# davidlougheed/strkit

Hardware: AMD Instinct MI355X
Metric: reads/sec realigned (higher is better)
Workload: dtype int32; 1 GPU; cfg2 shape (1000 loci x 30 HiFi reads, motif 3-6 bp, flank 70), 10000 loci x 30 reads per step and GPU, 8 distinct resident batches in rotation; exact scores (banded first pass with exactness certificate, exact fall-back); distinct_batches=8, parallelism=loci-sharded x1, calls_in_flight=2

## Files before the change

### strkit_amd/csrc/strk_api.hip

```cpp
#include "strk_host.h"
#include "strk_policy.h"
#include "strk_groups.h"
#include "strk_phase_check.h"
#include "strk_phase_inputs.h"
#include "strk_methyl.h"

#include <algorithm>
#include <array>
#include <atomic>
#include <chrono>
#include <cmath>
#include <condition_variable>
#include <cstdlib>
#include <cstring>
#include <memory>
#include <mutex>
#include <thread>
#include <vector>
#include <fcntl.h>
#include <sched.h>
#include <sys/stat.h>
#include <unistd.h>

#include "strk_kernels.h"
#include "strk_realign.h"
#include "strk_frontend.h"
#include "strk_inflate.h"
#include "strk_alleles.h"
#include "strk_phase.h"
#include "strk_consensus.h"
#include "strk_kmers.h"
#include "strk_poa.h"

namespace {

struct HostPipe;

std::atomic<int> g_calls_in_flight{0};

strk_policy::WindowPolicy g_window;
static_assert(strk_policy::kWinBuckets == strk::kWinBuckets, "strk_policy.h <-> strk_kernels.h");
static_assert(strk_groups::kInvalid == STRK_E_INVALID, "strk_groups.h <-> include/strkit_amd.h");
static_assert(strk_realign_plan::kNoMem == STRK_E_NOMEM, "strk_realign_plan.h <-> include/strkit_amd.h");

std::mutex g_band_chain_mu;
hipEvent_t g_band_chain_ev = nullptr;
int g_band_chain_dev = -1;

int host_cpus() {
    cpu_set_t set;
    CPU_ZERO(&set);
    if (sched_getaffinity(0, sizeof set, &set) == 0 && CPU_COUNT(&set) > 0) return CPU_COUNT(&set);
    return std::max(1u, std::thread::hardware_concurrency());
}

constexpr size_t kCellsOff = 64 * sizeof(int32_t);
constexpr size_t kCountersBytes = kCellsOff + 10 * sizeof(unsigned long long);
constexpr int kU64ScratchUsed = 1, kU64BandBytes = 2, kU64ExactBytes = 3, kU64WideBytes = 4, kU64LongBytes = 5;
constexpr size_t kWideHistOff = (kCountersBytes + 63) & ~(size_t)63;
constexpr size_t kCountersAllBytes = kWideHistOff + 2 * strk::kNumWideLists * 256 * sizeof(int32_t);

struct HostCounters {
    PinnedBuf mem;
    int cnt(int k) const { return mem.as<const int32_t>()[k]; }
    unsigned long long u64(int k) const { return reinterpret_cast<const unsigned long long*>(mem.as<const char>() + kCellsOff)[k]; }
    unsigned long long cells() const { return u64(0); }
    unsigned long long cells_of(int k_cell) const { return u64(k_cell); }
    unsigned long long scratch_used() const { return u64(kU64ScratchUsed); }
    unsigned long long band_bytes() const { return u64(kU64BandBytes); }
    unsigned long long exact_bytes() const { return u64(kU64ExactBytes); }
    unsigned long long wide_bytes() const { return u64(kU64WideBytes); }
    unsigned long long long_bytes() const { return u64(kU64LongBytes); }
    int band_reads() const {
        int n = 0;
        for (int k = 0; k < strk::kNumBandClasses; ++k) n += cnt(strk::kCntClass0 + strk::kBandClass0 + k);
        return n;
    }
};

struct GroupStage {
    DevBuf off, start, len, seqs;
    const uint8_t* bases = nullptr;
    int upload(const strk_groups::View& v, const strk_groups::Totals& t, const uint8_t* h_seqs, const uint8_t* d_seqs, hipStream_t st) {
        const size_t ng = (size_t)v.n_groups, ns = (size_t)t.n_seqs;
        int rc;
        if ((rc = off.ensure((ng + 1) * 4))) return rc;
        if ((rc = start.ensure(std::max<size_t>(ns, 1) * 8))) return rc;
        if ((rc = len.ensure(std::max<size_t>(ns, 1) * 4))) return rc;
        if (!d_seqs && (rc = seqs.ensure(std::max<size_t>((size_t)v.n_seq_bytes, 256)))) return rc;
        bases = d_seqs ? d_seqs : seqs.as<uint8_t>();
        if (!d_seqs && t.total_len > 0) HIP_TRY(hipMemcpyAsync(seqs.p, h_seqs, (size_t)v.n_seq_bytes, hipMemcpyHostToDevice, st));
        HIP_TRY(hipMemcpyAsync(off.p, v.group_off, (ng + 1) * 4, hipMemcpyHostToDevice, st));
        if (ns > 0) {
            HIP_TRY(hipMemcpyAsync(start.p, v.seq_start, ns * 8, hipMemcpyHostToDevice, st));
            HIP_TRY(hipMemcpyAsync(len.p, v.seq_len, ns * 4, hipMemcpyHostToDevice, st));
        }
        return 0;
    }
};

}

struct strk_ctx {
    int device = 0;
    int last_list_stride = 0;
    DevBuf read_locus, win_lo, win_n, tab_off, table, cls_list, band_recs, band_recs_w, long_list, counters, scratch, state_i32, state_f64, spec, rhash, rep, exact;
    DevBuf win_lo2, win_n2, tab_off2, table2, items;
    DevBuf stage_in, stage_out;
    PinnedBuf sc_host, sc_out;
    DevBuf rl_call, rl_chunk;
    Stream side;
    DevBuf al_in, al_ws, al_out;
    DevBuf ph_in, ph_mid, ph_ws, ph_out;
    GroupStage cs_in;
    DevBuf cs_bound, cs_out;
    GroupStage km_in;
    DevBuf km_k, km_cnt, km_eoff, km_list, km_slist, km_wsoff, km_ws, km_out;
    GroupStage po_in;
    DevBuf po_res, po_pool, po_poolof, po_list, po_ws, po_out, po_outoff;
    HostCounters h_counters;
    Event ev[9];
    size_t scratch_ints = 0;
    size_t long_slot_ints = 0, generic_ints = 0;
    strk_policy::BandGate band;
    strk_policy::GridHistory hist;
    bool p_window_auto = false;
    int p_window_b[strk::kWinBuckets] = {0, 0, 0, 0, 0};
    bool pending = false;
    strk_batch p_batch;
    strk_params p_params;
    strk_params p_params_in;
    int scratch_reruns = 0;
    strk::KArgs p_args;
    strk::ReplayArgs p_replay;
    hipStream_t p_stream = nullptr;
    HostPipe* pipe = nullptr;
};

namespace {

using namespace strk;

constexpr int kDefaultWindow = 8;
enum { kEvStart = 0, kEvHead, kEvBand, kEvWide, kEvPre, kEvExact, kEvLong, kEvGeneric, kEvEnd, kNumEvents };
constexpr int kBandProbationReads = 2048;
constexpr int kBandSpanW = 64, kBandSlackM8 = 0, kBandSpanMaxMotif = 6;
constexpr int kBandBlocksPerCU = std::max(1, std::min(8, (160 * 1024) / (4 * kBandWaveLds + kLdsSlack + 1024)));
constexpr int kLongBlocks = 512, kLongWaves = kLongBlocks * 4;
constexpr size_t kLongSlotInts = (size_t)48 << 10;
constexpr size_t kGenericPoolInts = (size_t)16 << 20;
constexpr size_t kLongSlotMaxInts = (size_t)kLongTile * kLongMaxTiles + 2 * (((size_t)1 << 20) + 256);
constexpr unsigned long long kGenericPoolMaxInts = 8ull << 30;
int check_params(const strk_params* p, strk_params* out) {
    if (!p) return fail(STRK_E_INVALID, "params is NULL");
    *out = *p;
    if (out->window <= 0) out->window = kDefaultWindow;
    if (2 * out->window + 1 > kTableMax) out->window = (kTableMax - 1) / 2;
    if (out->local_search_range < 0 || out->step_size < 1)
        return fail(STRK_E_INVALID, "local_search_range must be >= 0 and step_size >= 1");
    if (out->tie_rule != STRK_TIE_FIRST && out->tie_rule != STRK_TIE_LAST) return fail(STRK_E_INVALID, "bad tie_rule");
    if (out->end_flags < 0 || out->end_flags > 15) return fail(STRK_E_INVALID, "bad end_flags");
    static_assert(STRK_NARROW_NONE == strk::kNarrowNone && STRK_NARROW_DECREMENT == strk::kNarrowDecrement &&
                  STRK_NARROW_HALVE == strk::kNarrowHalve && STRK_NARROW_AFTER_SEED == strk::kNarrowAfterSeed, "include/strkit_amd.h <-> strk_search.h");
    if (out->narrowing < 0 || out->narrowing >= strk::kNarrowModes)
        return fail(STRK_E_INVALID, "narrowing schedule %d is not one of STRK_NARROW_NONE / _DECREMENT / _HALVE / _AFTER_SEED", out->narrowing);
    return 0;
}

int ensure_workspace(strk_ctx* c, int n_reads, int n_loci, size_t table_ints, size_t n_items) {
    const size_t nr = (size_t)std::max(n_reads, 1), nl = (size_t)std::max(n_loci, 1);
    int rc;
    if ((rc = c->read_locus.ensure(nr * 4))) return rc;
    if ((rc = c->win_lo.ensure(nr * 4))) return rc;
    if ((rc = c->win_n.ensure(nr * 4))) return rc;
    if ((rc = c->tab_off.ensure(nr * 8))) return rc;
    if ((rc = c->table.ensure(std::max<size_t>(table_ints, 1) * 4))) return rc;
    if ((rc = c->cls_list.ensure((size_t)kNumLists * std::max<size_t>(n_items, 1) * 2 * 4))) return rc;
    if ((rc = c->band_recs.ensure((size_t)kNumBandClasses * std::max<size_t>(n_items, 1) * 3 * sizeof(int4)))) return rc;
    if ((rc = c->counters.ensure(kCountersAllBytes))) return rc;
    if ((rc = c->band_recs_w.ensure((size_t)kNumBandClasses * std::max<size_t>(n_items, 1) * 3 * sizeof(int4)))) return rc;
    if ((rc = c->state_i32.ensure(nl * 4 * 4))) return rc;
    if ((rc = c->state_f64.ensure(nl * 8))) return rc;
    if ((rc = c->spec.ensure(nr * 16))) return rc;
    if ((rc = c->rhash.ensure(nr * 8))) return rc;
    if ((rc = c->rep.ensure(nr * 4))) return rc;
    if ((rc = c->exact.ensure(nr))) return rc;
    if (!c->scratch.p) {
        if ((rc = c->scratch.ensure(((size_t)kLongWaves * c->long_slot_ints + c->generic_ints) * 4))) return rc;
        c->scratch_ints = (size_t)kLongWaves * c->long_slot_ints + c->generic_ints;
    }
    return 0;
}

KArgs make_args(strk_ctx* c, const strk_batch* b, int end_flags, int window, int table_stride, int list_stride,
                const strk_params* sp) {
    KArgs a;
    memset(&a, 0, sizeof a);
    a.seqs = b->seqs; a.seq_off = b->seq_off; a.nfl = b->nfl; a.ntr = b->ntr; a.nfr = b->nfr;
    a.est_cn = b->est_cn; a.read_off = b->read_off; a.motifs = b->motifs; a.motif_off = b->motif_off;
    a.n_reads = b->n_reads; a.n_loci = b->n_loci;
    a.read_locus = c->read_locus.as<int32_t>();
    a.win_lo = c->win_lo.as<int32_t>();
    a.win_n = c->win_n.as<int32_t>();
    a.tab_off = c->tab_off.as<int64_t>();
    a.table = c->table.as<int32_t>();
    a.cls_list = c->cls_list.as<int32_t>();
    a.band_recs = c->band_recs.as<int4>();
    a.band_recs_w = a.band_recs;
    a.wide_hist = reinterpret_cast<int32_t*>(c->counters.as<char>() + kWideHistOff);
    a.counters = c->counters.as<int32_t>();
    a.cells = reinterpret_cast<unsigned long long*>(c->counters.as<char>() + kCellsOff);
    a.scratch_used = a.cells + 1;
    a.scratch = c->scratch.as<int32_t>();
    a.scratch_cap = (long long)c->scratch_ints;
    a.long_slot = (long long)c->long_slot_ints;
    a.long_waves = kLongWaves;
    a.list_stride = list_stride;
    c->last_list_stride = list_stride;
    a.band_tune = {kBandSpanW, kBandSlackM8, kBandSpanMaxMotif};
    a.end_flags = end_flags;
    a.window = window;
    for (int k = 0; k < kWinBuckets; ++k) a.window_b[k] = c->p_window_b[k] > 0 ? c->p_window_b[k] : window;
    a.table_stride = table_stride;
    if (sp) {
        a.spec = static_cast<int4*>(c->spec.p);
        a.max_iters = sp->max_iters; a.lsr = sp->local_search_range; a.step = sp->step_size;
        a.tie_last = sp->tie_rule == STRK_TIE_LAST;
        a.narrow = sp->narrowing;
        a.rep = c->rep.as<int32_t>();
        a.rhash = sp->no_dedupe ? nullptr : c->rhash.as<unsigned long long>();
        a.exact = c->exact.as<uint8_t>();
        a.band_mode = (!sp->no_band && c->band.cooldown == 0) ? 1 : 0;
        a.band_limit = c->band.probation ? kBandProbationReads : INT32_MAX;
    }
    return a;
}

void enqueue_scoring(strk_ctx* c, const KArgs& a, int mode, const int32_t* d_items, int n_items, int force_generic,
                     hipStream_t st, bool time_dp, const ReplayArgs* pre_replay = nullptr) {
    const bool hist = c->hist.usable(mode, a.band_mode);
    const bool sort_wide = a.band_mode && mode == 0 && !force_generic && (!hist || (c->hist.wide_chunks > 0 && c->hist.wide_chunks <= 8192));
    const int plan_scope = plan_scope_of(n_items);
    hipLaunchKernelGGL(k_plan, dim3((n_items + plan_scope - 1) / plan_scope), dim3(kPlanThreads), 0, st, a, mode, d_items, n_items, force_generic,
                       plan_reads_per_thread(n_items));
    const bool overlap = g_calls_in_flight.load(std::memory_order_relaxed) > 1;
    const bool heavy = c->hist.valid && c->hist.tail_heavy;
    const int sixteenths = (overlap && !heavy) ? 15 : 16;
    auto predicted_blocks = [&](int chunks, int full) { return c->hist.predicted_blocks(hist, chunks, a.n_reads, full); };
    if (time_dp) (void)hipEventRecord(c->ev[kEvHead], st);
    const bool band = a.band_mode && mode == 0 && !force_generic;
    int band_blocks = 1;
    if (band && time_dp) {
        std::lock_guard<std::mutex> lk(g_band_chain_mu);
        if (sixteenths == 16 && overlap && g_band_chain_ev && g_band_chain_ev != c->ev[kEvBand].h && g_band_chain_dev == c->device)
            (void)hipStreamWaitEvent(st, g_band_chain_ev, 0);
    }
    if (band) {
        band_blocks = std::max(1, std::min(256 * kBandBlocksPerCU * sixteenths / 16, (a.list_stride + 3) / 4));
        hipLaunchKernelGGL(k_dp_band, dim3(band_blocks), dim3(256), 0, st, a);
    }
    if (time_dp) (void)hipEventRecord(c->ev[kEvBand], st);
    if (band && time_dp) {
        std::lock_guard<std::mutex> lk(g_band_chain_mu);
        g_band_chain_ev = c->ev[kEvBand].h;
        g_band_chain_dev = c->device;
    }
    if (band) {
        KArgs aw = a;
        if (sort_wide) {
            hipLaunchKernelGGL(k_sort_wide_hist, dim3(kSortWideBlocks, kNumWideLists), dim3(256), 0, st, a);
            hipLaunchKernelGGL(k_sort_wide, dim3(kSortWideBlocks, kNumWideLists), dim3(256), 0, st, a, c->band_recs_w.as<int4>());
            aw.band_recs_w = c->band_recs_w.as<int4>();
        }
        const int wide_full = std::max(1, std::min(256 * kBandBlocksPerCU * sixteenths / 16, (a.list_stride + 3) / 4));
        hipLaunchKernelGGL(k_dp_band_wide, dim3(predicted_blocks(c->hist.wide_chunks, wide_full)), dim3(256), 0, st, aw);
    }
    if (time_dp) (void)hipEventRecord(c->ev[kEvWide], st);
    if (band && pre_replay) hipLaunchKernelGGL(k_replay, dim3(a.n_loci), dim3(64), 0, st, a, *pre_replay);
    if (time_dp) (void)hipEventRecord(c->ev[kEvPre], st);
    if (!force_generic) {
        constexpr int kBlocksPerCU = std::max(1, std::min(8, (160 * 1024) / (4 * kWaveLdsBytes + kLdsSlack + 1024)));
        const int full = std::max(1, std::min(256 * kBlocksPerCU * sixteenths / 16, (a.list_stride + 3) / 4));
        const int blocks = a.ref_mode ? full : predicted_blocks(c->hist.exact_chunks, full);
        if (a.ref_mode) hipLaunchKernelGGL(k_dp_ref, dim3(blocks), dim3(256), 0, st, a);
        else hipLaunchKernelGGL(k_dp_all, dim3(blocks), dim3(256), 0, st, a);
    }
    if (time_dp) (void)hipEventRecord(c->ev[kEvExact], st);
    KArgs al = a;
    if (!force_generic && !a.ref_mode) {
        const bool many_long = mode == 0 ? (!hist || c->hist.n_long > kLongWaves) : a.list_stride > kLongWaves;
        if (many_long && !c->long_list.ensure((size_t)std::max(1, a.list_stride) * 2 * 4)) {
            hipLaunchKernelGGL(k_sort_long, dim3(1), dim3(1024), 0, st, a, c->long_list.as<int32_t>());
            al.long_sorted = c->long_list.as<int32_t>();
        }
    }
    if (!force_generic && !a.ref_mode)
        hipLaunchKernelGGL(k_dp_long, dim3(mode == 0 ? predicted_blocks(c->hist.n_long, kLongBlocks) : std::max(1, std::min(kLongBlocks, a.list_stride))),
                           dim3(256), 0, st, al);
    if (time_dp) (void)hipEventRecord(c->ev[kEvLong], st);
    hipLaunchKernelGGL(k_dp_generic, dim3(1024), dim3(256), 0, st, a);
    if (time_dp) (void)hipEventRecord(c->ev[kEvGeneric], st);
}

// ... 30 lines not shown

int score_until_scratch_fits(strk_ctx* c, KArgs& a, const int32_t* d_items, int n_items, int force_generic, hipStream_t st,
                             bool timed, KArgs* outer = nullptr, void* copy_dst = nullptr, const void* copy_src = nullptr,
                             size_t copy_bytes = 0) {
    for (int attempt = 0;; ++attempt) {
        HIP_TRY(hipMemsetAsync(c->counters.p, 0, kCountersBytes, st));
        if (timed) HIP_TRY(hipEventRecord(c->ev[kEvStart], st));
        enqueue_scoring(c, a, 1, d_items, n_items, force_generic, st, timed);
        if (timed) HIP_TRY(hipEventRecord(c->ev[kEvEnd], st));
        HIP_TRY(hipMemcpyAsync(c->h_counters.mem.p, c->counters.p, kCountersBytes, hipMemcpyDeviceToHost, st));
        if (copy_bytes) HIP_TRY(hipMemcpyAsync(copy_dst, copy_src, copy_bytes, hipMemcpyDeviceToHost, st));
        HIP_TRY(hipStreamSynchronize(st));
        HIP_TRY(hipGetLastError());
        if (attempt >= 3 || !grow_scratch(c)) return 0;
        for (KArgs* k : {&a, outer}) {
            if (!k) continue;
            k->scratch = c->scratch.as<int32_t>();
            k->scratch_cap = (long long)c->scratch_ints;
            k->long_slot = (long long)c->long_slot_ints;
        }
    }
}

#include "strk_host_miss.inc"

int submit_device(strk_ctx* c, const strk_batch* b, const strk_params* params, int32_t* out_cn, int32_t* out_score,
                  int32_t* out_n, int32_t* out_start, hipStream_t st) {
    if (c->pending) return fail(STRK_E_INVALID, "context already holds a submitted call: strk_finish() it first");
    strk_params p;
    int rc;
    if ((rc = check_params(params, &p))) return rc;
    if (!b || b->n_reads < 0 || b->n_loci < 0) return fail(STRK_E_INVALID, "bad batch");
    c->p_window_auto = params->window <= 0;
    for (int k = 0; k < kWinBuckets; ++k) c->p_window_b[k] = 0;
    if (c->p_window_auto) {
        p.window = 0;
        for (int k = 0; k < kWinBuckets; ++k) {
            c->p_window_b[k] = g_window.window(k, p.local_search_range + p.step_size);
            p.window = std::max(p.window, c->p_window_b[k]);
        }
    }
    c->p_batch = *b;
    c->p_params = p;
    c->p_params_in = *params;
    c->p_stream = st;
    if (b->n_reads == 0 || b->n_loci == 0) {
        c->pending = true;
        g_calls_in_flight.fetch_add(1, std::memory_order_relaxed);
        return 0;
    }
    if (!out_cn || !out_score || !out_n || !out_start) return fail(STRK_E_INVALID, "output pointer is NULL");
    HIP_TRY(hipSetDevice(c->device));
    const int ts = std::min(kTableMax - 1, 2 * (p.window + 7) + 1);
    if ((rc = ensure_workspace(c, b->n_reads, b->n_loci, (size_t)b->n_reads * ts, (size_t)b->n_reads))) return rc;
    KArgs a = make_args(c, b, p.end_flags, p.window, ts, b->n_reads, &p);
    ReplayArgs rp;
    rp.max_iters = p.max_iters; rp.lsr = p.local_search_range; rp.step = p.step_size;
    rp.tie_last = p.tie_rule == STRK_TIE_LAST; rp.feedback = p.feedback; rp.narrow = p.narrowing;
    rp.out_cn = out_cn; rp.out_score = out_score; rp.out_n = out_n; rp.out_start = out_start;
    rp.next_read = c->state_i32.as<int32_t>();
    rp.need_lo = rp.next_read + b->n_loci;
    rp.need_hi = rp.need_lo + b->n_loci;
    rp.stop = rp.need_hi + b->n_loci;
    rp.frac = c->state_f64.as<double>();
    rp.resume = 0;
    rp.pre_exact = 0;

    struct InFlight {
        bool keep = false;
        InFlight() { g_calls_in_flight.fetch_add(1, std::memory_order_relaxed); }
        ~InFlight() { if (!keep) g_calls_in_flight.fetch_sub(1, std::memory_order_relaxed); }
    } in_flight;
    HIP_TRY(hipEventRecord(c->ev[kEvStart], st));
    HIP_TRY(hipMemsetAsync(c->counters.p, 0, kCountersAllBytes, st));
    if (a.rhash) hipLaunchKernelGGL(k_hash, dim3((b->n_reads + 31) / 32), dim3(256), 0, st, a);
    ReplayArgs rp_pre = rp;
    rp_pre.pre_exact = 1;
    enqueue_scoring(c, a, 0, nullptr, b->n_reads, 0, st, true, a.band_mode ? &rp_pre : nullptr);
    rp.resume = a.band_mode ? 1 : 0;
    hipLaunchKernelGGL(k_replay, dim3(b->n_loci), dim3(64), 0, st, a, rp);
    HIP_TRY(hipMemcpyAsync(c->h_counters.mem.p, c->counters.p, kCountersBytes, hipMemcpyDeviceToHost, st));
    HIP_TRY(hipEventRecord(c->ev[kEvEnd], st));
    HIP_TRY(hipGetLastError());
    c->p_args = a;
    c->p_replay = rp;
    c->pending = true;
    in_flight.keep = true;
    return 0;
}

void fill_stats(strk_ctx* c, const HostCounters& n, strk_stats* stats) {
    auto span = [&](int from, int to) {
        float ms = 0.f;
        return hipEventElapsedTime(&ms, c->ev[from], c->ev[to]) == hipSuccess ? ms : 0.f;
    };
    stats->kernel_ms = span(kEvStart, kEvEnd);
    stats->head_ms = span(kEvStart, kEvHead);
    stats->band_kernel_ms = span(kEvHead, kEvBand);
    stats->band_wide_kernel_ms = span(kEvBand, kEvWide);
    stats->dp_kernel_ms = span(kEvPre, kEvExact);
    stats->long_kernel_ms = span(kEvExact, kEvLong);
    stats->generic_kernel_ms = span(kEvLong, kEvGeneric);
    stats->replay_ms = span(kEvGeneric, kEvEnd) + span(kEvWide, kEvPre);
    stats->band_bytes = (int64_t)n.band_bytes();
    stats->exact_bytes = (int64_t)n.exact_bytes();
    stats->wide_bytes = (int64_t)n.wide_bytes();
    stats->long_bytes = (int64_t)n.long_bytes();
// ... 692 lines not shown
```

### strkit_amd/csrc/strk_dp_band.h

```cpp
#pragma once

namespace strk {

struct BandLayout {
    int wd, pad, maxdb, maxcol, off_sel, off_cp, cp_bytes, ct_bytes, cp_tail, off_ct, off_b0, group_bytes, sel_len;
    static constexpr int OFF_COMB = 0, OFF_MISC = OFF_COMB + kTableMax * 4, OFF_LMAX = OFF_MISC + 16;
    static constexpr int kBandHiPad = kBandRowSlack + 32;
    __host__ __device__ constexpr BandLayout(int c)
        : wd(128 << c), pad((128 << c) + (8 << c) + 8), maxdb(band_max_db(c)), maxcol(band_max_col(c)),
          off_sel(OFF_LMAX + (band_class_lmax(c) ? kTableMax * 4 : 0)),
          off_cp(off_sel + ((band_max_db(c) + 2 * ((128 << c) + (8 << c) + 8) + kBandHiPad + 15) & ~15)),
          cp_bytes(band_class_fly(c) ? 512 : ((band_max_db(c) + kBandRowSlack + 2 * (8 << c) + 4 + 15) & ~15)),
          ct_bytes((kBandMaxFlank + 2 * (8 << c) + 4 + 15) & ~15),
          cp_tail(c == 0 ? cp_bytes - ct_bytes : cp_bytes),
          off_ct(off_cp + cp_tail),
          off_b0(off_ct + ct_bytes),
          group_bytes(off_b0 + ((band_max_col(c) * 2 + 15) & ~15)),
          sel_len((band_max_db(c) + 2 * ((128 << c) + (8 << c) + 8) + kBandHiPad) & ~3) {}
};
static_assert(band_class_layout(4) == 0 && band_class_layout(7) == 3 && band_class_wd(5) <= band_class_wd(1) && band_class_G(6) == band_class_G(2),
              "a 12-diagonal class uses the LDS layout of the 16-diagonal class with its lane count: pads sized for the wider band cover it");
__host__ __device__ constexpr int band_wave_lds(int c) { return (64 / (8 << c)) * BandLayout(c).group_bytes; }
__host__ __device__ constexpr int max_band_wave_lds(int c) {
    return c < 0 ? 0 : (band_wave_lds(c) > max_band_wave_lds(c - 1) ? band_wave_lds(c) : max_band_wave_lds(c - 1));
// ... 317 lines not shown
        }
    }
    wave_lds_sync();
    {
        constexpr unsigned kNeg2 = ((unsigned)(unsigned short)(short)kBandNeg16) * 0x00010001u;
        const int nc2 = min(lay.maxcol, wave_max_over_groups(act ? geo.ncol : 0) + 1) >> 1;
        unsigned* const b2 = reinterpret_cast<unsigned*>(b0col);
        for (int k = lig; k <= nc2; k += G) if (2 * k < lay.maxcol) b2[k] = kNeg2;
    }
    wave_lds_sync();
    nextB();

    if (FLY) {
        const int rmax = wave_max_over_groups(rowsP);
        if (rmax >= 11264) __builtin_amdgcn_s_setprio(3);
        else if (rmax >= 8192) __builtin_amdgcn_s_setprio(2);
        else if (rmax >= 5120) __builtin_amdgcn_s_setprio(1);
    }
    BandCtx x;
    x.lig = lig; x.first = first; x.last = last; x.notFirst = first ? 0 : -1; x.notLast = last ? 0 : -1; x.selb = selb;
    asm volatile("" : "+v"(x.notFirst), "+v"(x.notLast));
    x.pad = lay.pad; x.maxidx = lay.sel_len - 1; x.ndb = ndb;
    x.flL = cp; x.motifL = motifL; x.nfl = nfl; x.m = m;
    x.flyP = FLY ? ((256 - 4) / m) * m : 0;
    const bool run = act && !fallback && geo.ok;
    const int nEff = run ? n : 0;
    x.tbl = s_tbl + kBandTblBytes;
    band_pass<G, D, true, false, false>(x, ct, run ? rowsT : 0, geo.bdlo, dbEnd, cEnd, 0, 0, 1, geo.cmin, geo.ncol, comb, b0col, lmaxA);
    wave_lds_sync();
    nextC();
    if (TAIL) {
        const int lenP = wave_max_over_groups(rowsP) + 2 * (G - 1) + 4;
        uint8_t* const cpr = cp + (G - 1);
        const uint8_t* const mo = a.motifs + misc[1];
        int mm = m, row0 = kRowTail + lig;
        asm volatile("" : "+v"(mm), "+v"(row0));
        for (int row = row0; row < lenP - (G - 1); row += G) {
            int sym = kNullSym;
            if (row < min(nfl, rowsP)) sym = kBandTblClass0 + selb[lay.pad + row];
            else if (row < rowsP) sym = s_enc[mo[(row - nfl) % mm]];
            cpr[row] = (uint8_t)(8 * sym);
        }
        wave_lds_sync();
    }
    x.tbl = s_tbl;
    band_pass<G, D, false, FLY, LMAX>(x, cp, run ? rowsP : 0, geo.dlo, dbBeg, cBeg, nEff, nfl + lo * m, m, geo.cmin, geo.ncol, comb, b0col, lmaxA);
    wave_lds_sync();
    if (FLY) __builtin_amdgcn_s_setprio(0);
    if (run) {
        for (int k = lig; k < n; k += G) {
            const int R = nfl + (lo + k) * m;
            int sc = max(comb[k], -(1 << 28)) - g * (R + nfr + ndb);
            if (LMAX && cEnd) sc = max(sc, max(lmaxA[k], -(1 << 28)) - g * ndb);
            comb[k] = sc;
            a.table[(long long)r * a.table_stride + k] = sc;
        }
    }
    int* const ubA = reinterpret_cast<int*>(b0col);
    if (run)
        for (int k = lig; k < n; k += G) ubA[k] = band_ub(geo, nfl, ntr, nfr, m, lo + k, a.end_flags);
    wave_lds_sync();
    if (act && first) {
        bool certified = false;
        if (run) {
            SeenMask64 seen;
            auto ub = [&](int k) { return ubA[k]; };
            const CertResult cr = search_replay_cert(q2.w, a.step, a.lsr, a.max_iters, a.tie_last, comb, lo, n, seen, ub, a.narrow);
            if (!cr.uncertain) {
                certified = true;
                a.spec[r] = make_int4(cr.res.cn, cr.res.score, cr.res.n_explored,
                                      (cr.res.miss ? kSpecMiss : 0) | (cr.res.empty ? kSpecEmpty : 0));
            }
        }
        if (!certified) {
            const int c = classify(nfl, ntr, nfr, m, lo, n, 0, 0);
            const int idx = atomicAdd(&a.counters[kCntClass0 + c], 1);
            if (idx < a.list_stride) {
                int32_t* gl = a.cls_list + (size_t)c * a.list_stride * 2;
                gl[2 * idx] = r;
                gl[2 * idx + 1] = 0;
            } else {
                atomicOr(&a.counters[kCntError], kErrList);
            }
            a.exact[r] = 1;
            atomicAdd(&a.counters[kCntBandFallback], 1);
            if (c != kGenericClass) {
                const unsigned long long cc = (unsigned long long)ndb * ((unsigned long long)nfl + (unsigned long long)(lo + n - 1) * m + nfr);
                atomicAdd(a.cells, cc);
                atomicAdd(a.cells + cell_slot_of_list(c), cc);
            }
        }
    }
    wave_lds_sync();
}

template <int SET>
__device__ __forceinline__ void band_kernel_body(const KArgs& a) {
    constexpr int C0 = SET ? 3 : 1, C1 = SET ? 7 : 5, C2 = SET ? 2 : 0, C3 = SET ? 6 : 4;
    const int n0_ = min(a.counters[kCntClass0 + kBandClass0 + C0], a.list_stride);
    const int n1_ = min(a.counters[kCntClass0 + kBandClass0 + C1], a.list_stride);
    const int n2_ = min(a.counters[kCntClass0 + kBandClass0 + C2], a.list_stride);
    const int n3_ = min(a.counters[kCntClass0 + kBandClass0 + C3], a.list_stride);
    if (n0_ + n1_ + n2_ + n3_ <= 0) return;
    constexpr int kTblBytes = 2 * kBandTblBytes;
    __shared__ __attribute__((aligned(16))) uint8_t lds[kTblBytes + 4 * kBandWaveLds + kLdsSlack];
    __shared__ uint8_t s_enc[256];
    static_assert(2 * (sizeof(lds) + 256) + 4608 <= 160 * 1024, "band kernels: two blocks per CU with room for k_plan's LDS");
    uint8_t* const s_tbl = lds;
    {
        s_enc[threadIdx.x] = c_enc[threadIdx.x];
        if (threadIdx.x < kTblBytes / 8) {
            const int pass = threadIdx.x / (kBandTblBytes / 8), t = threadIdx.x % (kBandTblBytes / 8);
            const bool topFree = a.end_flags & (pass ? 2 : 1), leftFree = a.end_flags & (pass ? 8 : 4);
            const int e = t < kBandTblClass0 ? t : (t < kBandTblClass0 + 8 ? band_class_symbol(t - kBandTblClass0) : -1);
            unsigned long long word = 0;
            for (int k = 0; k < 8; ++k) {
                const int cs = band_class_symbol(k);
                unsigned b = 0;
                if (t == kNullSym) {
                    b = (cs >= 0 && topFree) ? kGap : 0;
                } else if (e >= 0 && e < kNSym) {
                    if (cs >= 0) b = (unsigned)(c_mat[e][cs] + kWBias) & 0xffu;
                    else b = (leftFree && k == (pass ? kBandSelBack : kBandSelFront)) ? kGap : 0;
                }
                word |= (unsigned long long)b << (8 * k);
            }
            reinterpret_cast<unsigned long long*>(s_tbl)[threadIdx.x] = word;
        }
    }
    __syncthreads();
    uint8_t* const Lw = lds + kTblBytes + (threadIdx.x >> 6) * kBandWaveLds;
    constexpr int G01 = band_class_G(C0), G23 = band_class_G(C2);
    constexpr int per01 = 64 / G01, per23 = 64 / G23;
    const int ch0 = (n0_ + per01 - 1) / per01, ch1 = (n1_ + per01 - 1) / per01, ch2 = (n2_ + per23 - 1) / per23, ch3 = (n3_ + per23 - 1) / per23;
    const int e0 = ch0, e1 = e0 + ch1, e2 = e1 + ch2, e3 = e2 + ch3;
    const int lane = threadIdx.x & 63;
    auto pop = [&]() {
        int c = 0;
        if (lane == 0) c = atomicAdd(&a.counters[kCntNextBand + SET], 1);
        return __builtin_amdgcn_readfirstlane(c);
    };
    auto fetch = [&](int c, bool& act, int4& q0, int4& q1, int4& q2) -> int {
        int cls = C0, it = 0, cnt = 0, G_ = G01;
        if (c < e0) { cls = C0; it = c * per01 + lane / G01; cnt = n0_; }
// ... 51 lines not shown
```

### strkit_amd/csrc/strk_kernels.h

```cpp
#pragma once
#include <hip/hip_runtime.h>
#include <stdint.h>

#include "strk_scoring.h"
#include "strk_search.h"
#include "strk_plan_order.h"

namespace strk {

constexpr int kTableMax = 32;
static_assert(kTableMax < 64, "k_plan keeps a band item's table length in six bits");
constexpr int kNegInf = -(1 << 29);
constexpr int kFastFlankMax = 127;
constexpr int kMotifMax = 256;
constexpr int kRowSlack = 160;

constexpr int kNumClasses = 17;
__host__ __device__ constexpr int class_G(int c) { return c < 7 ? 8 : (c < 9 ? 16 : (c < 13 ? 32 : 64)); }
__host__ __device__ constexpr int class_CL(int c) {
    return c < 7 ? 16 + 4 * c : (c < 9 ? 24 + 4 * (c - 7) : (c < 13 ? 16 + 4 * (c - 9) : 16 + 4 * (c - 13)));
}
__host__ __device__ constexpr int class_cap(int c) { return class_G(c) * class_CL(c); }
constexpr int kLongClass = kNumClasses;
constexpr int kGenericClass = kNumClasses + 1;
constexpr int kBandClass0 = kNumClasses + 2;
constexpr int kNumLists = kNumClasses + 2 + kNumBandClasses;
constexpr int kLongTile = 64 * 28;
constexpr int kLongMaxTiles = 64;
constexpr int kLongFlankMax = 255;

__constant__ int8_t c_mat[kNSym][kNSym];
__constant__ uint8_t c_enc[256];

struct KArgs {
    const uint8_t* seqs;
    const int64_t* seq_off;
    const int32_t* nfl;
    const int32_t* ntr;
    const int32_t* nfr;
    const int32_t* est_cn;
    const int32_t* read_off;
    const uint8_t* motifs;
    const int32_t* motif_off;
    int32_t n_reads, n_loci;
    int32_t* read_locus;
    int32_t* win_lo;
    int32_t* win_n;
    int64_t* tab_off;
    int32_t* table;
    int32_t* cls_list;
    int4* band_recs;
    const int32_t* long_sorted;
    int4* band_recs_w;
    int32_t* wide_hist;
    int32_t* counters;
    unsigned long long* cells;
    int32_t* scratch;
    long long scratch_cap;
    unsigned long long* scratch_used;
    long long long_slot;
    int32_t long_waves;
    int4* spec;
    unsigned long long* rhash;
    int32_t* rep;
    int32_t list_stride;
    int32_t end_flags;
    int32_t window;
    int32_t window_b[5];
    int32_t table_stride;
    int32_t max_iters, lsr, step, tie_last;
    int32_t narrow;
    int32_t band_mode;
    int32_t band_limit;
    BandTune band_tune;
    uint8_t* exact;
    int32_t ref_mode;
};

enum Counter {
    kCntClass0 = 0,
    kCntMiss = kNumLists,
    kCntError = kNumLists + 1,
    kCntNextChunk = kNumLists + 2,
    kCntDup = kNumLists + 3,
    kCntNextLong = kNumLists + 4,
    kCntNextBand = kNumLists + 5,
    kCntBandFallback = kNumLists + 7,
    kCntMissB = kNumLists + 8,
    kCntLociB = kNumLists + 8 + 5,
    kCntTotal = kNumLists + 8 + 10,
    kCntLongNeed = 56
};
static_assert(kCntTotal <= 48 && kCntLongNeed < 64, "counters: 64 ints in front of the 64-bit counters; kCntLongNeed sits in the spare slots");
constexpr int kWinBuckets = 5;
__host__ __device__ constexpr int win_bucket(int m) { return m <= 2 ? 0 : (m <= 4 ? 1 : (m <= 6 ? 2 : (m <= 10 ? 3 : 4))); }
constexpr int kNumWideLists = 4;
__host__ __device__ constexpr int wide_slot(int band_cls) { return (band_cls & 1) | ((band_cls >> 2) << 1); }
__host__ __device__ constexpr int wide_slot_class(int slot) { return 2 + (slot & 1) + ((slot >> 1) << 2); }
__host__ __device__ constexpr int wide_bucket(int rows) { return rows >= (255 << 6) ? 255 : (rows < 0 ? 0 : rows >> 6); }
constexpr int kCellBand = 6, kCellWide = 7, kCellExact = 8, kCellLong = 9;
__host__ __device__ constexpr int cell_slot_of_list(int c) {
    return c >= kBandClass0 ? (band_class_wide_kernel(c - kBandClass0) ? kCellWide : kCellBand)
                            : (c == kLongClass ? kCellLong : (c == kGenericClass ? -1 : kCellExact));
}
constexpr int kErrBadInput = 1;
constexpr int kErrScratch = 2;
constexpr int kErrEmpty = 4;
constexpr int kErrList = 8;
constexpr int kErrLongSlot = 16;
constexpr int kSpecMiss = 1, kSpecEmpty = 2;

__device__ inline int classify(int nfl, int ntr, int nfr, int m, int lo, int n, int force_generic, int ref_mode) {
    const long long ndb = (long long)nfl + ntr + nfr;
    const long long rows = (long long)nfl + (long long)(lo + n - 1) * m;
    if (force_generic || nfl < 1 || (nfr < 1 && !ref_mode) || n > kTableMax || m > kMotifMax) return kGenericClass;
    for (int c = ref_mode ? kNumClasses - 1 : 0; c < kNumClasses; ++c) {
        const int cap = class_cap(c);
        if (ndb + 1 <= cap && rows <= cap + kRowSlack && (nfr <= kFastFlankMax || ref_mode)) return c;
    }
    if (!ref_mode && nfl <= kLongFlankMax && nfr <= kLongFlankMax && ndb + 1 <= (long long)kLongTile * kLongMaxTiles &&
        rows <= (1 << 20))
        return kLongClass;
    return kGenericClass;
}

__device__ __forceinline__ unsigned long long hash_mix(unsigned long long h, unsigned long long v) {
    h ^= v;
    h *= 0x9E3779B97F4A7C15ull;
    return h ^ (h >> 29);
}

__global__ void __launch_bounds__(256) k_hash(KArgs a) {
    const int gid = blockIdx.x * blockDim.x + threadIdx.x;
    const int r = gid >> 3, sl = gid & 7;
    const bool act = r < a.n_reads;
    unsigned long long h = 0xCBF29CE484222325ull + (unsigned long long)sl;
    if (act) {
        const uint8_t* p = a.seqs + a.seq_off[r];
        const int len = (int)(a.seq_off[r + 1] - a.seq_off[r]);
        const int nw = (len + 7) >> 3;
        for (int w = sl; w < nw; w += 8) {
            unsigned long long v = 0;
            const int i = w << 3;
            if (i + 8 <= len) __builtin_memcpy(&v, p + i, 8);
            else for (int k = 0; i + k < len; ++k) v |= (unsigned long long)p[i + k] << (8 * k);
            h = hash_mix(h, v + 0x9E3779B97F4A7C15ull * (unsigned long long)(w + 1));
        }
    }
#pragma unroll
    for (int o = 1; o < 8; o <<= 1) {
        const unsigned long long other = (unsigned long long)__shfl_down((long long)h, o, 8);
        h = hash_mix(h, other);
    }
    if (act && sl == 0) {
        h = hash_mix(h, ((unsigned long long)(unsigned)a.nfl[r] << 32) | (unsigned)a.ntr[r]);
        h = hash_mix(h, ((unsigned long long)(unsigned)a.nfr[r] << 32) | (unsigned)a.est_cn[r]);
        a.rhash[r] = h;
    }
}

__device__ inline bool same_read(const KArgs& a, int r, int q) {
    if (a.nfl[r] != a.nfl[q] || a.ntr[r] != a.ntr[q] || a.nfr[r] != a.nfr[q] || a.est_cn[r] != a.est_cn[q]) return false;
    const uint8_t* x = a.seqs + a.seq_off[r];
    const uint8_t* y = a.seqs + a.seq_off[q];
    const int len = a.nfl[r] + a.ntr[r] + a.nfr[r];
    int i = 0;
    for (; i + 32 <= len; i += 32) {
        unsigned long long u0, u1, u2, u3, v0, v1, v2, v3;
        __builtin_memcpy(&u0, x + i, 8); __builtin_memcpy(&u1, x + i + 8, 8); __builtin_memcpy(&u2, x + i + 16, 8); __builtin_memcpy(&u3, x + i + 24, 8);
        __builtin_memcpy(&v0, y + i, 8); __builtin_memcpy(&v1, y + i + 8, 8); __builtin_memcpy(&v2, y + i + 16, 8); __builtin_memcpy(&v3, y + i + 24, 8);
        if ((u0 ^ v0) | (u1 ^ v1) | (u2 ^ v2) | (u3 ^ v3)) return false;
    }
    for (; i + 8 <= len; i += 8) {
        unsigned long long u, v;
        __builtin_memcpy(&u, x + i, 8);
        __builtin_memcpy(&v, y + i, 8);
// ... 370 lines not shown
```

### strkit_amd/csrc/strk_replay.h

```cpp
#pragma once

namespace strk {

struct ReplayArgs {
    int32_t max_iters, lsr, step, tie_last, feedback, narrow;
    int32_t* out_cn;
    int32_t* out_score;
    int32_t* out_n;
    int32_t* out_start;
    int32_t* next_read;
    double* frac;
    int32_t* need_lo;
    int32_t* need_hi;
    int32_t pre_exact;
    int32_t resume;
    int32_t* stop;
};
constexpr int kStopNone = 0, kStopRescore = 1, kStopMiss = 2;

#ifndef STRK_REPLAY_WAVES
#define STRK_REPLAY_WAVES 5
#endif
__global__ void __launch_bounds__(64) __attribute__((amdgpu_waves_per_eu(STRK_REPLAY_WAVES, 8))) k_replay(KArgs a, ReplayArgs p) {
    const int l = blockIdx.x;
    const int lane = threadIdx.x;
    const int r_end = a.read_off[l + 1];
    double frac = 0.0;
    int r_next = a.read_off[l];
    if (p.resume) {
        if (p.stop[l] != kStopRescore) return;
        r_next = p.next_read[l];
        frac = p.frac[l];
    }
    bool missed = false, rescore = false;
    for (int base = r_next; base < r_end && !missed && !rescore; base += 64) {
        const int cnt = min(64, r_end - base);
        const int rl = base + lane;
        const int my_est = lane < cnt ? a.est_cn[rl] : 0;
        int4 my_spec = make_int4(0, 0, 0, kSpecMiss);
        if (a.spec && lane < cnt) my_spec = a.spec[a.rep[rl]];
        int o_cn = 0, o_score = 0, o_n = 0, o_start = 0;
        int done = 0;
        for (int i = 0; i < cnt; ++i) {
            const int est = __builtin_amdgcn_readlane(my_est, i);
            int start = est;
            double frac_try = frac;
            if (p.feedback) start = feedback_start(est, &frac_try);
            SearchResult res;
            const int spec_flags = __builtin_amdgcn_readlane(my_spec.w, i);
            if (start == est && !(spec_flags & kSpecMiss)) {
                res.cn = __builtin_amdgcn_readlane(my_spec.x, i);
                res.score = __builtin_amdgcn_readlane(my_spec.y, i);
                res.n_explored = __builtin_amdgcn_readlane(my_spec.z, i);
                res.miss = 0;
                res.empty = (spec_flags & kSpecEmpty) ? 1 : 0;
            } else {
                const int r = base + i;
                const int rp = a.rep[r];
                SeenMask64 seen;
                const bool is_exact = !a.band_mode || a.exact[rp];
                if (p.pre_exact && is_exact) {
                    rescore = true;
                    break;
                }
                if (is_exact) {
                    res = search_replay(start, p.step, p.lsr, p.max_iters, p.tie_last, a.table + a.tab_off[r], a.win_lo[r],
                                        min(a.win_n[r], 64), seen, p.narrow);
                } else {
                    const int nfl = a.nfl[rp], ntr = a.ntr[rp], nfr = a.nfr[rp];
                    const int m = a.motif_off[l + 1] - a.motif_off[l];
                    const int wlo = a.win_lo[r], wn = min(a.win_n[r], 64);
                    const BandGeo geo = band_geometry(nfl, ntr, nfr, m, wlo, wn, a.band_tune);
                    const int flags = a.end_flags;
                    auto ub = [&](int k) { return band_ub(geo, nfl, ntr, nfr, m, wlo + k, flags); };
                    const CertResult cr = search_replay_cert(start, p.step, p.lsr, p.max_iters, p.tie_last,
                                                             a.table + a.tab_off[r], wlo, wn, seen, ub, p.narrow);
                    res = cr.res;
                    if (cr.uncertain && p.pre_exact) {
                        for (int q0 = r; q0 < r_end; q0 += 64) {
                            const int q = q0 + lane;
                            if (q >= r_end) continue;
                            const int rq = a.rep[q];
                            unsigned* const w = reinterpret_cast<unsigned*>(a.exact + (rq & ~3));
                            const unsigned bit = 1u << (8 * (rq & 3));
                            if (atomicOr(w, bit) & (0xffu << (8 * (rq & 3)))) continue;
                            const int cls = classify(a.nfl[rq], a.ntr[rq], a.nfr[rq], m, a.win_lo[rq], min(a.win_n[rq], kTableMax), 0, 0);
                            const int idx = atomicAdd(&a.counters[kCntClass0 + cls], 1);
                            if (idx < a.list_stride) {
                                int32_t* gl = a.cls_list + (size_t)cls * a.list_stride * 2;
                                gl[2 * idx] = rq;
                                gl[2 * idx + 1] = 0;
                            } else {
                                atomicOr(&a.counters[kCntError], kErrList);
                            }
                            atomicAdd(&a.counters[kCntBandFallback], 1);
                            if (cls != kGenericClass) {
                                const unsigned long long cc = (unsigned long long)(a.nfl[rq] + a.ntr[rq] + a.nfr[rq]) *
                                                              ((unsigned long long)a.nfl[rq] + (unsigned long long)(a.win_lo[rq] + a.win_n[rq] - 1) * m + a.nfr[rq]);
                                atomicAdd(a.cells, cc);
                                atomicAdd(a.cells + cell_slot_of_list(cls), cc);
                            }
                        }
                        rescore = true;
                        break;
                    }
                    if (cr.uncertain) { res.miss = 1; res.need_lo = wlo; res.need_hi = wlo + wn - 1; }
                }
            }
            if (res.miss) {
                if (lane == 0) {
                    p.need_lo[l] = res.need_lo;
                    p.need_hi[l] = res.need_hi;
                    atomicAdd(&a.counters[kCntMiss], 1);
                }
                missed = true;
                break;
            }
            frac = frac_try;
            if (res.empty) {
                if (lane == 0) atomicOr(&a.counters[kCntError], kErrEmpty);
                res.cn = 0;
                res.score = 0;
            }
            if (lane == i) { o_cn = res.cn; o_score = res.score; o_n = res.n_explored; o_start = start; }
            if (p.feedback && !res.empty && res.cn != start) feedback_update(&frac, res.cn, start);
            done = i + 1;
        }
        if (lane < done) {
            p.out_cn[rl] = o_cn;
            p.out_score[rl] = o_score;
            p.out_n[rl] = o_n;
            p.out_start[rl] = o_start;
        }
        r_next = base + done;
    }
    if (lane == 0) {
        p.next_read[l] = r_next;
        p.frac[l] = frac;
        p.stop[l] = rescore ? kStopRescore : (missed ? kStopMiss : kStopNone);
        if (missed) atomicAdd(&a.counters[kCntMissB + win_bucket(a.motif_off[l + 1] - a.motif_off[l])], 1);
    }
}

}
```

### strkit_amd/csrc/strk_search.h

```cpp
#pragma once
#include <stdint.h>

#if defined(__HIPCC__)
#define STRK_HD __host__ __device__ inline
#else
#define STRK_HD inline
#endif

namespace strk {

struct SearchResult {
    int32_t cn, score, n_explored;
    int32_t miss;
    int32_t need_lo, need_hi;
    int32_t empty;
};

constexpr int32_t kNarrowNone = 0, kNarrowDecrement = 1, kNarrowHalve = 2, kNarrowAfterSeed = 3, kNarrowModes = 4;
struct LsrSchedule {
    int32_t mode, lsr, cur;
    STRK_HD LsrSchedule(int32_t mode_, int32_t lsr_) : mode(mode_), lsr(lsr_), cur(lsr_) {}
    STRK_HD int32_t floor1() const { return lsr < 1 ? lsr : 1; }
    STRK_HD int32_t at(bool seed) const { return mode == kNarrowAfterSeed ? (seed ? lsr : floor1()) : cur; }
    STRK_HD void explored() {
// ... 258 lines not shown
                    if (!have_best || s > best_s || (tie_last && s == best_s)) { have_best = true; best_i = (int32_t)i; best_s = s; }
                } else if (u > max_inexact) {
                    max_inexact = u;
                }
            }
            if (exact) {
                if (!have_mv || s > mv_s || (tie_last && s == mv_s)) { have_mv = true; mv_i = i; mv_s = s; }
            } else if (u > win_inexact) {
                win_inexact = u;
            }
        }
        if (!have_mv || win_inexact >= mv_s) { out.uncertain = 1; return out; }
        if (mv_i > size) {
            const int64_t nr = mv_i + step;
            const bool in_tab = nr >= lo && nr < (int64_t)lo + n;
            if (nr >= 0 && !(in_tab && seen.test((int32_t)(nr - lo)))) { st_size[sp] = nr; st_dir[sp++] = 1; }
        }
        if (mv_i < size) {
            const int64_t nr = mv_i - step;
            const bool in_tab = nr >= lo && nr < (int64_t)lo + n;
            if (nr >= 0 && !(in_tab && seen.test((int32_t)(nr - lo)))) { st_size[sp] = nr; st_dir[sp++] = -1; }
        }
    }
    res.n_explored = n_scored;
    if (n_scored == 0) { res.empty = 1; return out; }
    if (!have_best || max_inexact >= best_s) { out.uncertain = 1; return out; }
    res.cn = best_i;
    res.score = best_s;
    return out;
}

struct SeenMask64 {
    uint64_t m = 0;
    STRK_HD bool test(int k) const { return (m >> k) & 1; }
    STRK_HD void set(int k) { m |= (uint64_t)1 << k; }
};

STRK_HD int32_t feedback_start(int32_t est, double* frac) {
    int64_t sc = est;
#if defined(__HIP_DEVICE_COMPILE__)
    const int64_t off = (int64_t)rint(*frac * (double)sc);
#else
    const int64_t off = (int64_t)__builtin_rint(*frac * (double)sc);
#endif
    if (off < -sc) *frac = 0.0;
    else sc += off;
    return (int32_t)sc;
}

STRK_HD void feedback_update(double* frac, int32_t cn, int32_t start) {
    *frac += (double)(cn - start) / (double)(cn > 1 ? cn : 1);
}

}
```

Before: 283.0 million reads/s.

## Move band certification into replay and batch quiet reads with wave ballot

```diff
diff --git a/strkit_amd/csrc/strk_api.hip b/strkit_amd/csrc/strk_api.hip
--- a/strkit_amd/csrc/strk_api.hip
+++ b/strkit_amd/csrc/strk_api.hip
@@ -8,6 +8,7 @@
 #include <algorithm>
 #include <array>
 #include <atomic>
+#include <cassert>
 #include <chrono>
 #include <cmath>
 #include <condition_variable>
@@ -104,7 +105,7 @@
 struct strk_ctx {
     int device = 0;
     int last_list_stride = 0;
-    DevBuf read_locus, win_lo, win_n, tab_off, table, cls_list, band_recs, band_recs_w, long_list, counters, scratch, state_i32, state_f64, spec, rhash, rep, exact;
+    DevBuf read_locus, win_lo, win_n, tab_off, table, ub, cls_list, band_recs, band_recs_w, long_list, counters, scratch, state_i32, state_f64, spec, rhash, rep, exact;
     DevBuf win_lo2, win_n2, tab_off2, table2, items;
     DevBuf stage_in, stage_out;
     PinnedBuf sc_host, sc_out;
@@ -167,7 +168,7 @@
     return 0;
 }
 
-int ensure_workspace(strk_ctx* c, int n_reads, int n_loci, size_t table_ints, size_t n_items) {
+int ensure_workspace(strk_ctx* c, int n_reads, int n_loci, size_t table_ints, size_t n_items, bool band_tables = false) {
     const size_t nr = (size_t)std::max(n_reads, 1), nl = (size_t)std::max(n_loci, 1);
     int rc;
     if ((rc = c->read_locus.ensure(nr * 4))) return rc;
@@ -175,6 +176,7 @@
     if ((rc = c->win_n.ensure(nr * 4))) return rc;
     if ((rc = c->tab_off.ensure(nr * 8))) return rc;
     if ((rc = c->table.ensure(std::max<size_t>(table_ints, 1) * 4))) return rc;
+    if (band_tables && (rc = c->ub.ensure(std::max<size_t>(table_ints, 1) * 4))) return rc;
     if ((rc = c->cls_list.ensure((size_t)kNumLists * std::max<size_t>(n_items, 1) * 2 * 4))) return rc;
     if ((rc = c->band_recs.ensure((size_t)kNumBandClasses * std::max<size_t>(n_items, 1) * 3 * sizeof(int4)))) return rc;
     if ((rc = c->counters.ensure(kCountersAllBytes))) return rc;
@@ -204,6 +206,7 @@
     a.win_n = c->win_n.as<int32_t>();
     a.tab_off = c->tab_off.as<int64_t>();
     a.table = c->table.as<int32_t>();
+    a.ub = c->ub.as<int32_t>();
     a.cls_list = c->cls_list.as<int32_t>();
     a.band_recs = c->band_recs.as<int4>();
     a.band_recs_w = a.band_recs;
@@ -249,6 +252,7 @@
     auto predicted_blocks = [&](int chunks, int full) { return c->hist.predicted_blocks(hist, chunks, a.n_reads, full); };
     if (time_dp) (void)hipEventRecord(c->ev[kEvHead], st);
     const bool band = a.band_mode && mode == 0 && !force_generic;
+    assert(!band || (pre_replay && a.spec));
     int band_blocks = 1;
     if (band && time_dp) {
         std::lock_guard<std::mutex> lk(g_band_chain_mu);
@@ -385,7 +389,7 @@
     if (!out_cn || !out_score || !out_n || !out_start) return fail(STRK_E_INVALID, "output pointer is NULL");
     HIP_TRY(hipSetDevice(c->device));
     const int ts = std::min(kTableMax - 1, 2 * (p.window + 7) + 1);
-    if ((rc = ensure_workspace(c, b->n_reads, b->n_loci, (size_t)b->n_reads * ts, (size_t)b->n_reads))) return rc;
+    if ((rc = ensure_workspace(c, b->n_reads, b->n_loci, (size_t)b->n_reads * ts, (size_t)b->n_reads, !p.no_band))) return rc;
     KArgs a = make_args(c, b, p.end_flags, p.window, ts, b->n_reads, &p);
     ReplayArgs rp;
     rp.max_iters = p.max_iters; rp.lsr = p.local_search_range; rp.step = p.step_size;
diff --git a/strkit_amd/csrc/strk_dp_band.h b/strkit_amd/csrc/strk_dp_band.h
--- a/strkit_amd/csrc/strk_dp_band.h
+++ b/strkit_amd/csrc/strk_dp_band.h
@@ -393,44 +393,13 @@
             const int R = nfl + (lo + k) * m;
             int sc = max(comb[k], -(1 << 28)) - g * (R + nfr + ndb);
             if (LMAX && cEnd) sc = max(sc, max(lmaxA[k], -(1 << 28)) - g * ndb);
-            comb[k] = sc;
             a.table[(long long)r * a.table_stride + k] = sc;
-        }
-    }
-    int* const ubA = reinterpret_cast<int*>(b0col);
-    if (run)
-        for (int k = lig; k < n; k += G) ubA[k] = band_ub(geo, nfl, ntr, nfr, m, lo + k, a.end_flags);
-    wave_lds_sync();
-    if (act && first) {
-        bool certified = false;
-        if (run) {
-            SeenMask64 seen;
-            auto ub = [&](int k) { return ubA[k]; };
-            const CertResult cr = search_replay_cert(q2.w, a.step, a.lsr, a.max_iters, a.tie_last, comb, lo, n, seen, ub, a.narrow);
-            if (!cr.uncertain) {
-                certified = true;
-                a.spec[r] = make_int4(cr.res.cn, cr.res.score, cr.res.n_explored,
-                                      (cr.res.miss ? kSpecMiss : 0) | (cr.res.empty ? kSpecEmpty : 0));
-            }
-        }
-        if (!certified) {
-            const int c = classify(nfl, ntr, nfr, m, lo, n, 0, 0);
-            const int idx = atomicAdd(&a.counters[kCntClass0 + c], 1);
-            if (idx < a.list_stride) {
-                int32_t* gl = a.cls_list + (size_t)c * a.list_stride * 2;
-                gl[2 * idx] = r;
-                gl[2 * idx + 1] = 0;
-            } else {
-                atomicOr(&a.counters[kCntError], kErrList);
-            }
-            a.exact[r] = 1;
-            atomicAdd(&a.counters[kCntBandFallback], 1);
-            if (c != kGenericClass) {
-                const unsigned long long cc = (unsigned long long)ndb * ((unsigned long long)nfl + (unsigned long long)(lo + n - 1) * m + nfr);
-                atomicAdd(a.cells, cc);
-                atomicAdd(a.cells + cell_slot_of_list(c), cc);
-            }
-        }
+            a.ub[(long long)r * a.table_stride + k] = band_ub(geo, nfl, ntr, nfr, m, lo + k, a.end_flags);
+        }
+    }
+    if (act && first && !run) {
+        band_read_to_exact(a, r, nfl, ntr, nfr, m, lo, n);
+        a.exact[r] = 1;
     }
     wave_lds_sync();
 }
diff --git a/strkit_amd/csrc/strk_kernels.h b/strkit_amd/csrc/strk_kernels.h
--- a/strkit_amd/csrc/strk_kernels.h
+++ b/strkit_amd/csrc/strk_kernels.h
@@ -48,6 +48,7 @@
     int32_t* win_n;
     int64_t* tab_off;
     int32_t* table;
+    int32_t* ub;
     int32_t* cls_list;
     int4* band_recs;
     const int32_t* long_sorted;
@@ -108,7 +109,6 @@
 constexpr int kErrEmpty = 4;
 constexpr int kErrList = 8;
 constexpr int kErrLongSlot = 16;
-constexpr int kSpecMiss = 1, kSpecEmpty = 2;
 
 __device__ inline int classify(int nfl, int ntr, int nfr, int m, int lo, int n, int force_generic, int ref_mode) {
     const long long ndb = (long long)nfl + ntr + nfr;
@@ -122,6 +122,24 @@
         rows <= (1 << 20))
         return kLongClass;
     return kGenericClass;
+}
+
+__device__ inline void band_read_to_exact(const KArgs& a, int r, int nfl, int ntr, int nfr, int m, int lo, int n) {
+    const int c = classify(nfl, ntr, nfr, m, lo, n, 0, 0);
+    const int idx = atomicAdd(&a.counters[kCntClass0 + c], 1);
+    if (idx < a.list_stride) {
+        int32_t* gl = a.cls_list + (size_t)c * a.list_stride * 2;
+        gl[2 * idx] = r;
+        gl[2 * idx + 1] = 0;
+    } else {
+        atomicOr(&a.counters[kCntError], kErrList);
+    }
+    atomicAdd(&a.counters[kCntBandFallback], 1);
+    if (c != kGenericClass) {
+        const unsigned long long cc = (unsigned long long)(nfl + ntr + nfr) * ((unsigned long long)nfl + (unsigned long long)(lo + n - 1) * m + nfr);
+        atomicAdd(a.cells, cc);
+        atomicAdd(a.cells + cell_slot_of_list(c), cc);
+    }
 }
 
 __device__ __forceinline__ unsigned long long hash_mix(unsigned long long h, unsigned long long v) {
diff --git a/strkit_amd/csrc/strk_replay.h b/strkit_amd/csrc/strk_replay.h
--- a/strkit_amd/csrc/strk_replay.h
+++ b/strkit_amd/csrc/strk_replay.h
@@ -32,22 +32,66 @@
         r_next = p.next_read[l];
         frac = p.frac[l];
     }
+    if (p.pre_exact && a.band_mode && a.spec) {
+        const int m = a.motif_off[l + 1] - a.motif_off[l];
+        for (int base = r_next; base < r_end; base += 64) {
+            const int r = base + lane;
+            if (r >= r_end || a.rep[r] != r || a.exact[r]) continue;
+            const int wlo = a.win_lo[r], wn = min(a.win_n[r], 64);
+            const int32_t* const ubp = a.ub + a.tab_off[r];
+            SeenMask64 seen;
+            auto ub = [&](int k) { return ubp[k]; };
+            const CertResult cr = search_replay_cert(a.est_cn[r], p.step, p.lsr, p.max_iters, p.tie_last, a.table + a.tab_off[r],
+                                                     wlo, wn, seen, ub, p.narrow);
+            if (!cr.uncertain) {
+                a.spec[r] = make_int4(cr.res.cn, cr.res.score, cr.res.n_explored,
+                                      (cr.res.miss ? kSpecMiss : 0) | (cr.res.empty ? kSpecEmpty : 0));
+            } else {
+                band_read_to_exact(a, r, a.nfl[r], a.ntr[r], a.nfr[r], m, wlo, wn);
+                a.exact[r] = 1;
+            }
+        }
+        __builtin_amdgcn_fence(__ATOMIC_SEQ_CST, "workgroup");
+    }
     bool missed = false, rescore = false;
     for (int base = r_next; base < r_end && !missed && !rescore; base += 64) {
         const int cnt = min(64, r_end - base);
         const int rl = base + lane;
-        const int my_est = lane < cnt ? a.est_cn[rl] : 0;
-        int4 my_spec = make_int4(0, 0, 0, kSpecMiss);
-        if (a.spec && lane < cnt) my_spec = a.spec[a.rep[rl]];
-        int o_cn = 0, o_score = 0, o_n = 0, o_start = 0;
+        const unsigned ro = (unsigned)rl;
+        constexpr int kPendingBit = 4;
+        int my_est = 0, my_flags = kSpecMiss;
+        int4 my_spec = make_int4(0, 0, 0, 0);
+        if (lane < cnt) {
+            const int rp = a.rep[rl];
+            my_est = a.est_cn[rl];
+            if (a.spec) {
+                my_spec = a.spec[rp];
+                my_flags = my_spec.w;
+            }
+            if (p.pre_exact && (!a.band_mode || a.exact[rp])) my_flags |= kPendingBit;
+        }
         int done = 0;
-        for (int i = 0; i < cnt; ++i) {
+        while (done < cnt) {
+            const WalkRead rd = {my_est, my_spec.x, my_spec.y, my_spec.z, my_flags & (kSpecMiss | kSpecEmpty), my_flags & kPendingBit};
+            const bool quiet = lane < cnt && replay_quiet(rd, p.feedback, frac);
+            const unsigned long long loud = __builtin_amdgcn_ballot_w64(!quiet) & (~0ull << done);
+            const int ev = min(loud ? (int)__builtin_ctzll(loud) : 64, cnt);
+            if (lane >= done && lane < ev) {
+                p.out_cn[ro] = my_spec.x;
+                p.out_score[ro] = my_spec.y;
+                p.out_n[ro] = my_spec.z;
+                p.out_start[ro] = my_est;
+            }
+            done = ev;
+            if (ev >= cnt) break;
+            const int i = __builtin_amdgcn_readfirstlane(ev);
             const int est = __builtin_amdgcn_readlane(my_est, i);
             int start = est;
             double frac_try = frac;
             if (p.feedback) start = feedback_start(est, &frac_try);
+            start = __builtin_amdgcn_readfirstlane(start);
             SearchResult res;
-            const int spec_flags = __builtin_amdgcn_readlane(my_spec.w, i);
+            const int spec_flags = __builtin_amdgcn_readlane(my_flags, i);
             if (start == est && !(spec_flags & kSpecMiss)) {
                 res.cn = __builtin_amdgcn_readlane(my_spec.x, i);
                 res.score = __builtin_amdgcn_readlane(my_spec.y, i);
@@ -67,12 +111,10 @@
                     res = search_replay(start, p.step, p.lsr, p.max_iters, p.tie_last, a.table + a.tab_off[r], a.win_lo[r],
                                         min(a.win_n[r], 64), seen, p.narrow);
                 } else {
-                    const int nfl = a.nfl[rp], ntr = a.ntr[rp], nfr = a.nfr[rp];
                     const int m = a.motif_off[l + 1] - a.motif_off[l];
                     const int wlo = a.win_lo[r], wn = min(a.win_n[r], 64);
-                    const BandGeo geo = band_geometry(nfl, ntr, nfr, m, wlo, wn, a.band_tune);
-                    const int flags = a.end_flags;
-                    auto ub = [&](int k) { return band_ub(geo, nfl, ntr, nfr, m, wlo + k, flags); };
+                    const int32_t* const ubp = a.ub + a.tab_off[r];
+                    auto ub = [&](int k) { return ubp[k]; };
                     const CertResult cr = search_replay_cert(start, p.step, p.lsr, p.max_iters, p.tie_last,
                                                              a.table + a.tab_off[r], wlo, wn, seen, ub, p.narrow);
                     res = cr.res;
@@ -84,22 +126,7 @@
                             unsigned* const w = reinterpret_cast<unsigned*>(a.exact + (rq & ~3));
                             const unsigned bit = 1u << (8 * (rq & 3));
                             if (atomicOr(w, bit) & (0xffu << (8 * (rq & 3)))) continue;
-                            const int cls = classify(a.nfl[rq], a.ntr[rq], a.nfr[rq], m, a.win_lo[rq], min(a.win_n[rq], kTableMax), 0, 0);
-                            const int idx = atomicAdd(&a.counters[kCntClass0 + cls], 1);
-                            if (idx < a.list_stride) {
-                                int32_t* gl = a.cls_list + (size_t)cls * a.list_stride * 2;
-                                gl[2 * idx] = rq;
-                                gl[2 * idx + 1] = 0;
-                            } else {
-                                atomicOr(&a.counters[kCntError], kErrList);
-                            }
-                            atomicAdd(&a.counters[kCntBandFallback], 1);
-                            if (cls != kGenericClass) {
-                                const unsigned long long cc = (unsigned long long)(a.nfl[rq] + a.ntr[rq] + a.nfr[rq]) *
-                                                              ((unsigned long long)a.nfl[rq] + (unsigned long long)(a.win_lo[rq] + a.win_n[rq] - 1) * m + a.nfr[rq]);
-                                atomicAdd(a.cells, cc);
-                                atomicAdd(a.cells + cell_slot_of_list(cls), cc);
-                            }
+                            band_read_to_exact(a, rq, a.nfl[rq], a.ntr[rq], a.nfr[rq], m, a.win_lo[rq], min(a.win_n[rq], kTableMax));
                         }
                         rescore = true;
                         break;
@@ -122,15 +149,14 @@
                 res.cn = 0;
                 res.score = 0;
             }
-            if (lane == i) { o_cn = res.cn; o_score = res.score; o_n = res.n_explored; o_start = start; }
+            if (lane == i) {
+                p.out_cn[ro] = res.cn;
+                p.out_score[ro] = res.score;
+                p.out_n[ro] = res.n_explored;
+                p.out_start[ro] = start;
+            }
             if (p.feedback && !res.empty && res.cn != start) feedback_update(&frac, res.cn, start);
             done = i + 1;
-        }
-        if (lane < done) {
-            p.out_cn[rl] = o_cn;
-            p.out_score[rl] = o_score;
-            p.out_n[rl] = o_n;
-            p.out_start[rl] = o_start;
         }
         r_next = base + done;
     }
diff --git a/strkit_amd/csrc/strk_search.h b/strkit_amd/csrc/strk_search.h
--- a/strkit_amd/csrc/strk_search.h
+++ b/strkit_amd/csrc/strk_search.h
@@ -334,4 +334,114 @@
     *frac += (double)(cn - start) / (double)(cn > 1 ? cn : 1);
 }
 
-}
+constexpr int32_t kSpecMiss = 1, kSpecEmpty = 2;
+
+struct WalkRead {
+    int32_t est;
+    int32_t cn, score, n_explored;
+    int32_t flags;
+    int32_t pending;
+};
+struct WalkOut {
+    int32_t cn, score, n_explored, start;
+};
+constexpr int32_t kWalkNext = 0, kWalkRescore = 1, kWalkMiss = 2;
+
+STRK_HD bool same_double_bits(double x, double y) {
+    uint64_t a, b;
+    __builtin_memcpy(&a, &x, 8);
+    __builtin_memcpy(&b, &y, 8);
+    return a == b;
+}
+
+STRK_HD bool replay_quiet(const WalkRead& rd, int32_t feedback, double frac) {
+    if (rd.flags != 0) return false;
+    if (!feedback) return true;
+    if (rd.pending) return false;
+    double f = frac;
+    const int32_t start = feedback_start(rd.est, &f);
+    return start == rd.est && same_double_bits(f, frac) && rd.cn == start;
+}
+
+template <class Search>
+STRK_HD int32_t replay_walk_step(const WalkRead& rd, int32_t i, int32_t feedback, int32_t pre_exact, double* frac, WalkOut* out,
+                                 const Search& search) {
+    int32_t start = rd.est;
+    double frac_try = *frac;
+    if (feedback) start = feedback_start(rd.est, &frac_try);
+    SearchResult res = {0, 0, 0, 0, 0, 0, 0};
+    if (start == rd.est && !(rd.flags & kSpecMiss)) {
+        res.cn = rd.cn;
+        res.score = rd.score;
+        res.n_explored = rd.n_explored;
+        res.empty = (rd.flags & kSpecEmpty) ? 1 : 0;
+    } else {
+        if (pre_exact && rd.pending) return kWalkRescore;
+        int32_t uncertain = 0;
+        res = search(i, start, &uncertain);
+        if (uncertain && pre_exact) return kWalkRescore;
+        if (uncertain) res.miss = 1;
+    }
+    if (res.miss) return kWalkMiss;
+    *frac = frac_try;
+    if (res.empty) {
+        res.cn = 0;
+        res.score = 0;
+    }
+    out->cn = res.cn;
+    out->score = res.score;
+    out->n_explored = res.n_explored;
+    out->start = start;
+    if (feedback && !res.empty && res.cn != start) feedback_update(frac, res.cn, start);
+    return kWalkNext;
+}
+
+template <class Search>
+STRK_HD int32_t replay_walk_serial(const WalkRead* rd, int32_t n, int32_t feedback, int32_t pre_exact, double* frac, WalkOut* out,
+                                   int32_t* next, const Search& search) {
+    int32_t i = 0, how = kWalkNext;
+    for (; i < n; ++i) {
+        how = replay_walk_step(rd[i], i, feedback, pre_exact, frac, out + i, search);
+        if (how != kWalkNext) break;
+    }
+    *next = i;
+    return how;
+}
+
+template <class Search, class OnEvent>
+STRK_HD int32_t replay_walk_events(const WalkRead* rd, int32_t n, int32_t feedback, int32_t pre_exact, double* frac, WalkOut* out,
+                                   int32_t* next, const Search& search, const OnEvent& on_event) {
+    int32_t done_all = 0, how = kWalkNext;
+    for (int32_t base = 0; base < n && how == kWalkNext; base += 64) {
+        const int32_t cnt = n - base < 64 ? n - base : 64;
+        int32_t pos = 0;
+        while (pos < cnt) {
+            uint64_t loud = 0;
+            for (int32_t j = 0; j < 64; ++j)
+                if (j >= cnt || !replay_quiet(rd[base + j], feedback, *frac)) loud |= (uint64_t)1 << j;
+            loud &= ~(uint64_t)0 << pos;
+            int32_t ev = 64;
+            for (int32_t j = 0; j < 64 && ev == 64; ++j)
+                if ((loud >> j) & 1) ev = j;
+            if (ev > cnt) ev = cnt;
+            for (int32_t j = pos; j < ev; ++j) {
+                const WalkRead& q = rd[base + j];
+                out[base + j].cn = q.cn;
+                out[base + j].score = q.score;
+                out[base + j].n_explored = q.n_explored;
+                out[base + j].start = q.est;
+            }
+            pos = ev;
+            if (ev >= cnt) break;
+            on_event(ev, base);
+            how = replay_walk_step(rd[base + ev], base + ev, feedback, pre_exact, frac, out + base + ev, search);
+            if (how != kWalkNext) break;
+            pos = ev + 1;
+        }
+        done_all = base + pos;
+    }
+    *next = done_all;
+    return how;
+}
+
+}
```

Result: faster. 311.0 million reads/s (median of 6 runs) (+9.9%).
